# HaploConduct/HaploConduct

Hardware: NVIDIA B200
Metric: candidate_overlaps_scored_per_sec (higher is better)
Workload: dtype u32 fixed-point (2^-22) sums + f64 reference-order pass at threshold boundaries

## Files before the change

### haploconduct_b200/csrc/hc_kernels.cu

```cuda
#include "hc_kernels.cuh"

namespace {

typedef unsigned long long u64;

struct Win {
    u64 xpos;
    uint32_t ypos16;
    uint32_t L;
    uint32_t status;
    uint32_t hasN;
};

struct CandSetup {
    Win w[2];
    uint32_t two;
    uint32_t err;
};

__device__ __forceinline__ hc_candidate load_candidate(const hc_kparams& P, u64 i) {
    hc_candidate c;
    if (P.cand_compact == 4u) {
        const uint16_t* hp = reinterpret_cast<const uint16_t*>(P.cand) + 3 * i;
        const uint32_t h0 = __ldg(hp), h1 = __ldg(hp + 1), h2 = __ldg(hp + 2);
        const uint32_t lo = h0 | (h1 << 16);
        uint32_t r = __ldg(P.tile_run + (i >> 5));
        while ((uint32_t)i >= __ldg(P.run_start + r + 1)) r++;
        const uint32_t anchor = __ldg(P.run_anchor + r), other = lo & 0x01ffffffu;
        const bool anchor_is_2 = ((lo >> 25) & 1u) != 0u;
        c.idx1 = anchor_is_2 ? other : anchor;
        c.idx2 = anchor_is_2 ? anchor : other;
        c.pos1 = (lo >> 30) | ((h2 & 0x7fu) << 2);
        c.pos2 = h2 >> 7;
        c.len1 = c.len2 = 0; c.perc1 = c.perc2 = 0; c.type1 = c.type2 = 0; c.reserved = 0;
        c.ori1 = (lo >> 26) & 1u; c.ori2 = (lo >> 27) & 1u;
        const uint32_t o = (lo >> 28) & 3u;
        c.ord = o == 1 ? '1' : (o == 2 ? '2' : '-');
        return c;
    }
    if (P.cand_compact == 3u) {
        const uint2 e = __ldg(reinterpret_cast<const uint2*>(P.cand) + i);
        uint32_t r = __ldg(P.tile_run + (i >> 5));
        while ((uint32_t)i >= __ldg(P.run_start + r + 1)) r++;
        const uint32_t anchor = __ldg(P.run_anchor + r), other = e.x & 0x7fffffffu;
        const bool anchor_is_2 = (e.x >> 31) != 0u;
        c.idx1 = anchor_is_2 ? other : anchor;
        c.idx2 = anchor_is_2 ? anchor : other;
        const uint32_t w = e.y;
        c.pos1 = w & 0x3fffu; c.pos2 = (w >> 14) & 0x3fffu;
        c.len1 = c.len2 = 0; c.perc1 = c.perc2 = 0; c.type1 = c.type2 = 0; c.reserved = 0;
        c.ori1 = (w >> 28) & 1u; c.ori2 = (w >> 29) & 1u;
        const uint32_t o = w >> 30;
        c.ord = o == 1 ? '1' : (o == 2 ? '2' : '-');
        return c;
    }
    if (P.cand_compact == 2u) {
        const uint32_t* sp = reinterpret_cast<const uint32_t*>(P.cand) + 3 * i;
        const uint32_t w = __ldg(sp + 2);
        c.idx1 = __ldg(sp); c.idx2 = __ldg(sp + 1); c.pos1 = w & 0x3fffu; c.pos2 = (w >> 14) & 0x3fffu;
        c.len1 = c.len2 = 0; c.perc1 = c.perc2 = 0; c.type1 = c.type2 = 0; c.reserved = 0;
        c.ori1 = (w >> 28) & 1u; c.ori2 = (w >> 29) & 1u;
        const uint32_t o = w >> 30;
        c.ord = o == 1 ? '1' : (o == 2 ? '2' : '-');
        return c;
    }
    if (P.cand_compact) {
        const uint4 a = __ldg(reinterpret_cast<const uint4*>(P.cand) + i);
        c.idx1 = a.x; c.idx2 = a.y; c.pos1 = a.z & 0x0fffffffu; c.pos2 = a.w;
        c.len1 = c.len2 = 0; c.perc1 = c.perc2 = 0; c.type1 = c.type2 = 0; c.reserved = 0;
        c.ori1 = (a.z >> 28) & 1u; c.ori2 = (a.z >> 29) & 1u;
        const uint32_t o = a.z >> 30;
        c.ord = o == 1 ? '1' : (o == 2 ? '2' : '-');
        return c;
    }
    const uint4* cp = reinterpret_cast<const uint4*>(P.cand) + 2 * i;
    const uint4 a = __ldg(cp), b = __ldg(cp + 1);
    c.idx1 = a.x; c.idx2 = a.y; c.pos1 = a.z; c.pos2 = a.w;
    c.len1 = b.x; c.len2 = b.y;
    c.perc1 = b.z & 0xff; c.perc2 = (b.z >> 8) & 0xff; c.ord = (b.z >> 16) & 0xff; c.ori1 = (b.z >> 24) & 0xff;
    c.ori2 = b.w & 0xff; c.type1 = (b.w >> 8) & 0xff; c.type2 = (b.w >> 16) & 0xff; c.reserved = 0;
    return c;
}

__device__ __forceinline__ void make_window(const hc_kparams& P, uint32_t rawA, uint32_t slotA, int rcA, uint32_t rawB,
                                            uint32_t slotB, int rcB, uint32_t pos, Win& w) {
    const uint32_t lenA = rawA & HC_LEN_MASK, lenB = rawB & HC_LEN_MASK;
    w.L = 0;
    w.xpos = 0;
    w.ypos16 = 0;
    w.hasN = 0;
    if (pos >= lenA) { w.status = HC_WIN_POS_OOR; return; }
    if (lenA < P.min_read_len || lenB < P.min_read_len) { w.status = HC_WIN_SHORT; return; }
    const u64 sa = 16ull * slotA + (rcA ? hc_slot_size(lenA) : 0u);
    const u64 sb = 16ull * slotB + (rcB ? hc_slot_size(lenB) : 0u);
    w.xpos = sa + pos;
    w.ypos16 = (uint32_t)(sb >> 4);
    w.L = min(lenA - pos, lenB);
    w.status = HC_WIN_SCORED;
    w.hasN = ((rawA | rawB) & HC_HASN_BIT) ? 1u : 0u;
}

__device__ __forceinline__ void setup_windows(const hc_kparams& P, const hc_candidate& c, const uint4& r1, const uint4& r2,
                                              CandSetup& s) {
    const int p1 = (r1.w & HC_LEN_MASK) != 0, p2 = (r2.w & HC_LEN_MASK) != 0;
    const int rc1 = c.ori1 ? 0 : 1, rc2 = c.ori2 ? 0 : 1;
    const int f1 = p1 ? rc1 : 0, s1 = p1 ? 1 - rc1 : 0;
    const int f2 = p2 ? rc2 : 0, s2 = p2 ? 1 - rc2 : 0;
    s.two = (p1 | p2) ? 1u : 0u;
    s.err = 0;
    s.w[1].L = 0; s.w[1].xpos = 0; s.w[1].ypos16 = 0; s.w[1].hasN = 0; s.w[1].status = HC_WIN_UNUSED;
    if (p1 && p2) { if (c.ord != '1' && c.ord != '2') s.err = 1; }
    else if (P.n_single == 0) s.err = 1;
    make_window(P, f1 ? r1.w : r1.z, f1 ? r1.y : r1.x, rc1, f2 ? r2.w : r2.z, f2 ? r2.y : r2.x, rc2, c.pos1, s.w[0]);
    if (s.two) {
        const uint32_t ra = s1 ? r1.w : r1.z, sa = s1 ? r1.y : r1.x;
        const uint32_t rb = s2 ? r2.w : r2.z, sb = s2 ? r2.y : r2.x;
        const bool swapped = p1 && (!p2 || c.ord == '2');
        if (swapped) make_window(P, rb, sb, rc2, ra, sa, rc1, c.pos2, s.w[1]);
        else make_window(P, ra, sa, rc1, rb, sb, rc2, c.pos2, s.w[1]);
    }
    if (s.err) { s.w[0].L = s.w[1].L = 0; s.w[0].status = s.w[1].status = HC_WIN_UNUSED; }
}

__device__ __forceinline__ void extra_pos(const hc_candidate& c, const uint4& r1, const uint4& r2, int32_t& pos3, int32_t& pos4) {
    const uint32_t l10 = r1.z & HC_LEN_MASK, l11 = r1.w & HC_LEN_MASK, l20 = r2.z & HC_LEN_MASK, l21 = r2.w & HC_LEN_MASK;
    const int p1 = l11 != 0, p2 = l21 != 0;
    if (!p1 && !p2) { pos3 = (int32_t)(l10 - c.pos1 - l20); pos4 = 0; }
    else if (!p1) { pos3 = (int32_t)(l10 - c.pos2 - l21); pos4 = (int32_t)(l10 - c.pos1 - l20); }
    else if (!p2) { pos3 = (int32_t)(l11 + c.pos2 - l20); pos4 = (int32_t)(l20 + c.pos1 - l10); }
    else {
        pos3 = c.ord == '1' ? (int32_t)(l11 - c.pos2 - l21) : (int32_t)(l11 + c.pos2 - l21);
        pos4 = (int32_t)(l10 - c.pos1 - l20);
    }
}

__device__ __forceinline__ bool load_and_setup(const hc_kparams& P, const hc_candidate& c, CandSetup& s, uint4& r1, uint4& r2) {
    if (c.idx1 >= P.n_reads || c.idx2 >= P.n_reads || c.idx1 == c.idx2) {
        s.err = 1; s.two = 0;
        s.w[0].L = s.w[1].L = 0; s.w[0].xpos = s.w[1].xpos = 0; s.w[0].ypos16 = s.w[1].ypos16 = 0;
        s.w[0].hasN = s.w[1].hasN = 0; s.w[0].status = s.w[1].status = HC_WIN_UNUSED;
        r1 = r2 = make_uint4(0, 0, 0, 0);
        return false;
    }
    r1 = __ldg(reinterpret_cast<const uint4*>(P.rdesc + c.idx1));
    r2 = __ldg(reinterpret_cast<const uint4*>(P.rdesc + c.idx2));
    setup_windows(P, c, r1, r2, s);
    return !s.err;
}

__device__ __forceinline__ void prefetch_l2(const void* p) { asm volatile("prefetch.global.L2 [%0];" ::"l"(p)); }

__device__ __forceinline__ void prefetch_window(const hc_kparams& P, const Win& w) {
    if (w.L == 0) return;
    const uint32_t n = min(w.L, 512u);
    if (P.packed) {
        const uint8_t* xa = P.pk + (w.xpos & ~127ull);
        const uint32_t xe = (uint32_t)(w.xpos & 127ull) + n;
        for (uint32_t o = 0; o < xe; o += 128) prefetch_l2(xa + o);
        const uint8_t* ya = P.pk + 16ull * w.ypos16;
        for (uint32_t o = 0; o < n; o += 128) prefetch_l2(ya + o);
        return;
    }
    const uint8_t* xa = P.qual + (w.xpos & ~127ull);
    const uint32_t xe = (uint32_t)(w.xpos & 127ull) + n;
    for (uint32_t o = 0; o < xe; o += 128) prefetch_l2(xa + o);
    const uint8_t* ya = P.qual + 16ull * w.ypos16;
    for (uint32_t o = 0; o < n; o += 128) prefetch_l2(ya + o);
    prefetch_l2(P.base2 + (w.xpos >> 4));
    prefetch_l2(P.base2 + ((w.xpos + n) >> 4));
    prefetch_l2(P.base2 + w.ypos16);
}

__device__ __forceinline__ uint32_t prmt(uint32_t a, uint32_t b, uint32_t sel) {
    uint32_t d;
    asm("prmt.b32 %0, %1, %2, %3;" : "=r"(d) : "r"(a), "r"(b), "r"(sel));
    return d;
}

__device__ __forceinline__ void ldg256(const void* p, uint32_t* d) {
    asm("ld.global.nc.v8.u32 {%0,%1,%2,%3,%4,%5,%6,%7}, [%8];"
        : "=r"(d[0]), "=r"(d[1]), "=r"(d[2]), "=r"(d[3]), "=r"(d[4]), "=r"(d[5]), "=r"(d[6]), "=r"(d[7])
        : "l"(p));
}

template <bool HAS_VOID>
__device__ __forceinline__ void lookup16(const uint32_t* __restrict__ T, const uint32_t* wa, const uint32_t* wy, uint32_t m,
                                         uint32_t& acc, uint32_t& orv) {
#pragma unroll
    for (int j = 0; j < 4; j++) {
        const uint32_t mj = (m >> (8 * j)) & 0x55u;
        const uint32_t dep = (mj * 0x02082080u) & 0x80808080u;
        const uint32_t col = (wa[j] ^ hc_swz4(wy[j])) | dep;
        const uint32_t t0 = T[prmt(col, wy[j], 0xCC40u)];
        const uint32_t t1 = T[prmt(col, wy[j], 0xDD51u)];
        const uint32_t t2 = T[prmt(col, wy[j], 0xEE62u)];
        const uint32_t t3 = T[prmt(col, wy[j], 0xFF73u)];
        acc += (t0 + t1) + (t2 + t3);
        if (HAS_VOID) orv |= (t0 | t1) | (t2 | t3);
    }
}

template <bool HAS_VOID>
__device__ __forceinline__ void process32(const hc_kparams& P, const uint32_t* __restrict__ T, u64 xpos, uint32_t ypos16,
                                          uint32_t L, uint32_t hasN, uint32_t k, uint32_t& sum, uint32_t& mm, uint32_t& ncnt,
                                          uint32_t& vd) {
    const u64 xp = xpos + 32ull * k;
    const uint32_t n = min(L - 32u * k, 32u);
    const uint32_t yq = ypos16 + 2u * k;
    const uint32_t off = (uint32_t)xp & 15u;
    const bool two = n > 16u, x1 = off + n > 16u, x2 = off + n > 32u;
    const uint4 z4 = make_uint4(0, 0, 0, 0);
#ifndef HC_NO_LD256
    const uint32_t off32 = (uint32_t)xp & 31u;
    uint32_t QA[16], wy[8];
    const uint8_t* xb = P.qual + (xp & ~31ull);
    ldg256(xb, QA);
    if (off32 + n > 32u) ldg256(xb + 32, QA + 8);
    else {
#pragma unroll
        for (int i = 8; i < 16; i++) QA[i] = 0u;
    }
    ldg256(P.qual + 16ull * yq, wy);
    (void)two; (void)z4;
#else
    const uint4* xq = reinterpret_cast<const uint4*>(P.qual + (xp & ~15ull));
    const uint4 q0 = __ldg(xq);
    const uint4 q1 = x1 ? __ldg(xq + 1) : z4;
    const uint4 q2 = x2 ? __ldg(xq + 2) : z4;
    const uint4* yqp = reinterpret_cast<const uint4*>(P.qual) + yq;
    const uint4 y0 = __ldg(yqp);
    const uint4 y1 = two ? __ldg(yqp + 1) : z4;
#endif
    const uint32_t* bxp = P.base2 + (xp >> 4);
    const uint32_t b0 = __ldg(bxp);
    const uint32_t b1 = x1 ? __ldg(bxp + 1) : 0u;
    const uint32_t b2 = x2 ? __ldg(bxp + 2) : 0u;
    const uint2 by = __ldg(reinterpret_cast<const uint2*>(P.base2 + yq));
    const uint32_t bsh = off * 2u;
    const uint32_t xa0 = __funnelshift_r(b0, b1, bsh) ^ by.x;
    const uint32_t xa1 = __funnelshift_r(b1, b2, bsh) ^ by.y;
    uint32_t m0 = (xa0 | (xa0 >> 1)) & 0x55555555u;
    uint32_t m1 = (xa1 | (xa1 >> 1)) & 0x55555555u;
    if (n < 32u) {
        const uint32_t n0 = min(n, 16u), n1 = n - n0;
        m0 &= n0 >= 16u ? 0xffffffffu : ((1u << (2u * n0)) - 1u);
        m1 &= (1u << (2u * n1)) - 1u;
    }
    ncnt = 0;
    if (hasN) {
        const uint32_t* nap = P.nmask + (xp >> 5);
        const uint32_t na0 = __ldg(nap), na1 = __ldg(nap + 1);
        uint32_t nn = __funnelshift_r(na0, na1, (uint32_t)xp & 31u) | __ldg(P.nmask + (yq >> 1));
        if (n < 32u) nn &= (1u << n) - 1u;
        ncnt = __popc(nn);
        uint32_t s0 = nn & 0xffffu, s1 = nn >> 16;
        s0 = (s0 | (s0 << 8)) & 0x00ff00ffu; s1 = (s1 | (s1 << 8)) & 0x00ff00ffu;
        s0 = (s0 | (s0 << 4)) & 0x0f0f0f0fu; s1 = (s1 | (s1 << 4)) & 0x0f0f0f0fu;
        s0 = (s0 | (s0 << 2)) & 0x33333333u; s1 = (s1 | (s1 << 2)) & 0x33333333u;
        s0 = (s0 | (s0 << 1)) & 0x55555555u; s1 = (s1 | (s1 << 1)) & 0x55555555u;
        m0 &= ~s0;
        m1 &= ~s1;
    }
    mm = __popc(m0) + __popc(m1);
    const bool s2 = (off & 8u) != 0, s1 = (off & 4u) != 0;
    uint32_t V1[10], V[9];
#ifndef HC_NO_LD256
    const bool s4 = (off32 & 16u) != 0;
    uint32_t V2[12];
#pragma unroll
    for (int i = 0; i < 12; i++) V2[i] = s4 ? QA[i + 4] : QA[i];
#pragma unroll
    for (int i = 0; i < 10; i++) V1[i] = s2 ? V2[i + 2] : V2[i];
#else
    const uint32_t W[12] = {q0.x, q0.y, q0.z, q0.w, q1.x, q1.y, q1.z, q1.w, q2.x, q2.y, q2.z, q2.w};
#pragma unroll
    for (int i = 0; i < 10; i++) V1[i] = s2 ? W[i + 2] : W[i];
    const uint32_t wy[8] = {y0.x, y0.y, y0.z, y0.w, y1.x, y1.y, y1.z, y1.w};
#endif
#pragma unroll
    for (int i = 0; i < 9; i++) V[i] = s1 ? V1[i + 1] : V1[i];
    const uint32_t sh = (off & 3u) * 8u;
    uint32_t wa[8];
#pragma unroll
    for (int i = 0; i < 8; i++) wa[i] = __funnelshift_r(V[i], V[i + 1], sh);
    uint32_t acc = 0, orv = 0;
    lookup16<HAS_VOID>(T, wa, wy, m0, acc, orv);
    lookup16<HAS_VOID>(T, wa + 4, wy + 4, m1, acc, orv);
    sum = acc;
    vd = HAS_VOID ? ((orv & HC_VOID_BIT) ? 1u : 0u) : 0u;
}

#ifdef HC_NO_LD256
struct PkRow {
    uint4 q0, q1, q2, y0, y1;
    uint32_t n, off, hasN;
};
#else
struct PkRow {
    uint32_t a[16];
    uint32_t y[8];
    uint32_t n, off, hasN;
};

#endif

__device__ __forceinline__ PkRow load32_packed(const hc_kparams& P, u64 xpos, uint32_t ypos16, uint32_t L, uint32_t hasN, uint32_t k) {
    PkRow r;
    const u64 xp = xpos + 32ull * k;
    r.n = min(L - 32u * k, 32u);
    const uint32_t yq = ypos16 + 2u * k;
    r.hasN = hasN;
#ifndef HC_NO_LD256
    r.off = (uint32_t)xp & 31u;
    const uint8_t* xb = P.pk + (xp & ~31ull);
    ldg256(xb, r.a);
    if (r.off + r.n > 32u) ldg256(xb + 32, r.a + 8);
    else {
#pragma unroll
        for (int i = 8; i < 16; i++) r.a[i] = 0u;
    }
    ldg256(P.pk + 16ull * yq, r.y);
    return r;
#else
    r.off = (uint32_t)xp & 15u;
    const bool two = r.n > 16u, x1 = r.off + r.n > 16u, x2 = r.off + r.n > 32u;
    const uint4 z4 = make_uint4(0, 0, 0, 0);
    const uint4* xq = reinterpret_cast<const uint4*>(P.pk + (xp & ~15ull));
    r.q0 = __ldg(xq);
    r.q1 = x1 ? __ldg(xq + 1) : z4;
    r.q2 = x2 ? __ldg(xq + 2) : z4;
    const uint4* yqp = reinterpret_cast<const uint4*>(P.pk) + yq;
    r.y0 = __ldg(yqp);
    r.y1 = two ? __ldg(yqp + 1) : z4;
    return r;
#endif
}

template <bool HAS_VOID>
__device__ __forceinline__ void compute32_packed(const uint32_t* __restrict__ T, const uint32_t* __restrict__ VM, const PkRow& r,
                                                 uint32_t& sum, uint32_t& mm, uint32_t& ncnt, uint32_t& vd) {
    const uint32_t n = r.n, off = r.off, hasN = r.hasN;
    const uint32_t vm = VM[n];
#ifndef HC_NO_LD256
    const bool s4 = (off & 16u) != 0, s2 = (off & 8u) != 0, s1 = (off & 4u) != 0;
    uint32_t V2[12], V1[10], V[9];
#pragma unroll
    for (int i = 0; i < 12; i++) V2[i] = s4 ? r.a[i + 4] : r.a[i];
#pragma unroll
    for (int i = 0; i < 10; i++) V1[i] = s2 ? V2[i + 2] : V2[i];
#pragma unroll
    for (int i = 0; i < 9; i++) V[i] = s1 ? V1[i + 1] : V1[i];
    const uint32_t sh = (off & 3u) * 8u;
    const uint32_t* wy = r.y;
#else
    const uint4 q0 = r.q0, q1 = r.q1, q2 = r.q2, y0 = r.y0, y1 = r.y1;
    const uint32_t W[12] = {q0.x, q0.y, q0.z, q0.w, q1.x, q1.y, q1.z, q1.w, q2.x, q2.y, q2.z, q2.w};
    const bool s2 = (off & 8u) != 0, s1 = (off & 4u) != 0;
    uint32_t V1[10], V[9];
#pragma unroll
    for (int i = 0; i < 10; i++) V1[i] = s2 ? W[i + 2] : W[i];
#pragma unroll
    for (int i = 0; i < 9; i++) V[i] = s1 ? V1[i + 1] : V1[i];
    const uint32_t sh = (off & 3u) * 8u;
    const uint32_t wy[8] = {y0.x, y0.y, y0.z, y0.w, y1.x, y1.y, y1.z, y1.w};
#endif
    uint32_t acc = 0, orv = 0, flags = 0, vw = 0;
#pragma unroll
    for (int j = 0; j < 8; j++) {
        const uint32_t wa = __funnelshift_r(V[j], V[j + 1], sh);
        const uint32_t wb = wy[j];
        const uint32_t col = wa ^ hc_swz4_packed(wb);
        const uint32_t row = wb & 0x3f3f3f3fu;
        flags |= ((col | (col << 1)) & 0x80808080u) >> j;
        if (hasN) {
            const uint32_t nzA = (((wa & 0x7f7f7f7fu) + 0x7f7f7f7fu) | wa), nzB = (((wb & 0x7f7f7f7fu) + 0x7f7f7f7fu) | wb);
            vw |= ((nzA & nzB) & 0x80808080u) >> j;
        }
        const uint32_t t0 = T[prmt(col, row, 0xCC40u)];
        const uint32_t t1 = T[prmt(col, row, 0xDD51u)];
        const uint32_t t2 = T[prmt(col, row, 0xEE62u)];
        const uint32_t t3 = T[prmt(col, row, 0xFF73u)];
        acc += (t0 + t1) + (t2 + t3);
        if (HAS_VOID) orv |= (t0 | t1) | (t2 | t3);
    }
    ncnt = 0;
    if (hasN) {
        const uint32_t valid = vw & vm;
        ncnt = n - __popc(valid);
        flags &= valid;
    } else {
        flags &= vm;
    }
    mm = __popc(flags);
    sum = acc;
    vd = HAS_VOID ? ((orv & HC_VOID_BIT) ? 1u : 0u) : 0u;
}

template <bool HAS_VOID>
__device__ __forceinline__ void process32_packed(const hc_kparams& P, const uint32_t* __restrict__ T,
                                                 const uint32_t* __restrict__ VM, u64 xpos, uint32_t ypos16, uint32_t L,
                                                 uint32_t hasN, uint32_t k, uint32_t& sum, uint32_t& mm, uint32_t& ncnt,
                                                 uint32_t& vd) {
    const PkRow r = load32_packed(P, xpos, ypos16, L, hasN, k);
    compute32_packed<HAS_VOID>(T, VM, r, sum, mm, ncnt, vd);
}

template <bool HAS_VOID, bool PACKED>
__device__ __forceinline__ void process_chunk(const hc_kparams& P, const uint32_t* __restrict__ T, const uint32_t* __restrict__ VM,
                                              u64 xpos, uint32_t ypos16, uint32_t L, uint32_t hasN, uint32_t k, uint32_t& sum,
                                              uint32_t& mm, uint32_t& ncnt, uint32_t& vd) {
    if (PACKED) process32_packed<HAS_VOID>(P, T, VM, xpos, ypos16, L, hasN, k, sum, mm, ncnt, vd);
    else process32<HAS_VOID>(P, T, xpos, ypos16, L, hasN, k, sum, mm, ncnt, vd);
}

__device__ __forceinline__ uint32_t warp_incl_scan(uint32_t v, int lane) {
#pragma unroll
    for (int d = 1; d < 32; d <<= 1) {
        uint32_t t = __shfl_up_sync(0xffffffffu, v, d);
        if (lane >= d) v += t;
    }
    return v;
}

struct WinAcc {
    u64 S;
    uint32_t mm;
    uint32_t nn;
    uint32_t vd;
};

__device__ __forceinline__ double window_mm_rate(uint32_t mm, uint32_t tl) {
    if (tl == 0u) return 1.0;
    return mm ? (double)(float)(int)mm / (double)tl : 0.0;
}

__device__ __forceinline__ uint32_t classify(const hc_kparams& P, uint32_t two, const uint32_t mmc[2], const uint32_t cmp[2],
                                             const int ae[2], const int ao[2]) {
    int both, ov_ok;
    if (two) {
        both = ae[0] && ae[1];
        ov_ok = ao[0] && ao[1];
    } else {
        both = ae[0];
        ov_ok = ao[0];
    }
    uint32_t cls;
    if (both) cls = HC_CLASS_EDGE;
    else {
        bool low;
        if (P.merge_contigs_sign == 0) low = cmp[0] != 0u && mmc[0] == 0u && (!two || (cmp[1] != 0u && mmc[1] == 0u));
        else if (P.merge_contigs_sign < 0) low = false;
        else {
            const double r0 = window_mm_rate(mmc[0], cmp[0]), r1 = window_mm_rate(mmc[1], cmp[1]);
            low = (two ? fmax(r0, r1) : r0) <= P.merge_contigs;
        }
        if (low) cls = HC_CLASS_EDGE;
        else if (ov_ok) cls = HC_CLASS_NONEDGE;
        else cls = HC_CLASS_DISCARD;
    }
    return cls | (both ? HC_CLS_BOTH : 0u);
}

__device__ __forceinline__ double combine_score(uint32_t two, uint32_t both, double ov0, double ov1) {
    if (!two) return ov0;
    return both ? 0.5 * (ov0 + ov1) : fmin(ov0, ov1);
}

__device__ __forceinline__ double fx_mean(u64 S, uint32_t tl) { return -((double)S * (1.0 / HC_FX_SCALE)) / (double)tl; }

__device__ __noinline__ void write_per_cand(const hc_kparams& P, u64 i, double score, double mmrate, uint32_t cls,
                                            const uint32_t mmc[2], const uint32_t cmp[2], const uint32_t st[2], uint32_t exact) {
    hc_result r;
    r.score = score;
    r.mismatch_rate = mmrate;
    const hc_candidate c = load_candidate(P, i);
    uint4 r1 = make_uint4(0, 0, 0, 0), r2 = r1;
    if (c.idx1 < P.n_reads && c.idx2 < P.n_reads) {
        r1 = __ldg(reinterpret_cast<const uint4*>(P.rdesc + c.idx1));
        r2 = __ldg(reinterpret_cast<const uint4*>(P.rdesc + c.idx2));
    }
    extra_pos(c, r1, r2, r.pos3, r.pos4);
    r.mismatches[0] = mmc[0];
    r.mismatches[1] = mmc[1];
    r.compared[0] = cmp[0];
    r.compared[1] = cmp[1];
    r.cls = (uint8_t)(cls & HC_CLS_MASK);
    r.status[0] = (uint8_t)st[0];
    r.status[1] = (uint8_t)st[1];
    r.exact = (uint8_t)exact;
    r.indel_count = 0;
    P.per_cand[i] = r;
}

template <bool HAS_VOID, bool PACKED>
__global__ void __launch_bounds__(HC_WARPS_MAX * 32, HC_MIN_CTAS) hc_score_kernel(const hc_kparams P) {
    extern __shared__ __align__(16) unsigned char smem[];
    uint32_t* T = reinterpret_cast<uint32_t*>(smem);
    const uint32_t ntab = (P.ncodes + 1u) * 256u;
    uint32_t* VM = T + ntab;
    for (uint32_t i = threadIdx.x; i < ntab; i += blockDim.x) T[i] = P.fx_table[i];
    if (threadIdx.x < HC_VM_WORDS) VM[threadIdx.x] = hc_packed_vmask(threadIdx.x);
    __syncthreads();

    const int lane = threadIdx.x & 31;
    const int warp = threadIdx.x >> 5;
    const int nwarps = blockDim.x >> 5;
    unsigned char* scratch = smem + (size_t)(ntab + HC_VM_WORDS) * 4u + (size_t)warp * HC_WARP_SCRATCH;
    uint2* part = reinterpret_cast<uint2*>(scratch);
    uint4* wdA = reinterpret_cast<uint4*>(scratch + HC_PARTMAX * 8u);
    uint2* wdB = reinterpret_cast<uint2*>(scratch + HC_PARTMAX * 8u + HC_WINSLOTS * 16u);
    uint32_t* head = reinterpret_cast<uint32_t*>(scratch + HC_PARTMAX * 8u + HC_WINSLOTS * 24u);

    const u64 ntiles = (P.n + 31ull) >> 5;
    const u64 gwarp = (u64)blockIdx.x * nwarps + warp;
    const u64 twarps = (u64)gridDim.x * nwarps;
    const uint32_t lane_le = 0xffffffffu >> (31 - lane);

    uint32_t st_windows = 0, st_positions = 0, st_bytes = 0, st_errors = 0;

    for (u64 tile = gwarp; tile < ntiles; tile += twarps) {
        const u64 i = (tile << 5) + lane;
        const bool valid = i < P.n;
        CandSetup s;
        s.err = 0; s.two = 0;
        s.w[0].L = s.w[1].L = 0; s.w[0].status = s.w[1].status = HC_WIN_UNUSED;
        s.w[0].xpos = s.w[1].xpos = 0; s.w[0].ypos16 = s.w[1].ypos16 = 0; s.w[0].hasN = s.w[1].hasN = 0;
        if (valid) {
            const hc_candidate c = load_candidate(P, i);
            uint4 r1, r2;
            load_and_setup(P, c, s, r1, r2);
#ifndef HC_NO_PREFETCH
            prefetch_window(P, s.w[0]);
            prefetch_window(P, s.w[1]);
#endif
        }
        WinAcc acc[2];
        acc[0].S = acc[1].S = 0; acc[0].mm = acc[1].mm = 0; acc[0].nn = acc[1].nn = 0; acc[0].vd = acc[1].vd = 0;
        const uint32_t c0 = (s.w[0].L + 31u) >> 5, c1 = (s.w[1].L + 31u) >> 5;
        const uint32_t ct = c0 + c1;

        uint32_t bigmask = __ballot_sync(0xffffffffu, ct >= HC_BIG_CHUNKS);
        while (bigmask) {
            const int src = __ffs(bigmask) - 1;
            bigmask &= bigmask - 1;
#pragma unroll
            for (int w = 0; w < 2; w++) {
                const uint32_t xl = __shfl_sync(0xffffffffu, (uint32_t)s.w[w].xpos, src);
                const uint32_t xh = __shfl_sync(0xffffffffu, (uint32_t)(s.w[w].xpos >> 32), src);
                const uint32_t yp = __shfl_sync(0xffffffffu, s.w[w].ypos16, src);
                const uint32_t Lw = __shfl_sync(0xffffffffu, s.w[w].L, src);
                const uint32_t hn = __shfl_sync(0xffffffffu, s.w[w].hasN, src);
                const uint32_t cw = (Lw + 31u) >> 5;
                if (cw == 0) continue;
                const u64 xpos = ((u64)xh << 32) | xl;
                u64 S = 0;
                uint32_t mm = 0, nn = 0, vd = 0;
                for (uint32_t k = lane; k < cw; k += 32) {
                    uint32_t sum, m1, n1, v1;
                    process_chunk<HAS_VOID, PACKED>(P, T, VM, xpos, yp, Lw, hn, k, sum, m1, n1, v1);
                    S += sum; mm += m1; nn += n1; vd |= v1;
                }
#pragma unroll
                for (int d = 16; d > 0; d >>= 1) {
                    S += __shfl_xor_sync(0xffffffffu, S, d);
                    mm += __shfl_xor_sync(0xffffffffu, mm, d);
                    nn += __shfl_xor_sync(0xffffffffu, nn, d);
                    vd |= __shfl_xor_sync(0xffffffffu, vd, d);
                }
                if (lane == src) { acc[w].S = S; acc[w].mm = mm; acc[w].nn = nn; acc[w].vd = vd; }
            }
        }

        uint32_t pending = __ballot_sync(0xffffffffu, ct > 0 && ct < HC_BIG_CHUNKS);
        while (pending) {
            const bool mine = (pending >> lane) & 1u;
            const uint32_t nwin = (c0 > 0) + (c1 > 0);
            const uint32_t v = mine ? (ct | (nwin << 16)) : 0u;
            const uint32_t incl = warp_incl_scan(v, lane);
            const bool fit = mine && ((incl & 0xffffu) <= HC_PARTMAX);
            const uint32_t take = __ballot_sync(0xffffffffu, fit);
            const int last = 31 - __clz(take);
            const uint32_t C = __shfl_sync(0xffffffffu, incl, last) & 0xffffu;
            if (lane < (int)(HC_PARTMAX / 32u)) head[lane] = 0;
            __syncwarp();
            uint32_t start0 = 0, start1 = 0;
            if (fit) {
                start0 = (incl & 0xffffu) - ct;
                start1 = start0 + c0;
                uint32_t slot = (incl >> 16) - nwin;
                if (c0) {
                    wdA[slot] = make_uint4((uint32_t)s.w[0].xpos, (uint32_t)(s.w[0].xpos >> 32), s.w[0].ypos16, s.w[0].L);
                    wdB[slot] = make_uint2(start0, s.w[0].hasN);
                    atomicOr(&head[start0 >> 5], 1u << (start0 & 31u));
                    slot++;
                }
                if (c1) {
                    wdA[slot] = make_uint4((uint32_t)s.w[1].xpos, (uint32_t)(s.w[1].xpos >> 32), s.w[1].ypos16, s.w[1].L);
                    wdB[slot] = make_uint2(start1, s.w[1].hasN);
                    atomicOr(&head[start1 >> 5], 1u << (start1 & 31u));
                }
            }
            __syncwarp();
            uint32_t running = 0;
            for (uint32_t f0 = 0; f0 < C; f0 += 32) {
                const uint32_t hw = head[f0 >> 5];
                const uint32_t f = f0 + lane;
                if (f < C) {
                    const uint32_t slot = running + __popc(hw & lane_le) - 1u;
                    const uint4 a = wdA[slot];
                    const uint2 b = wdB[slot];
                    uint32_t sum, m1, n1, v1;
                    process_chunk<HAS_VOID, PACKED>(P, T, VM, ((u64)a.y << 32) | a.x, a.z, a.w, b.y, f - b.x, sum, m1, n1, v1);
                    part[f] = make_uint2(sum, m1 | (n1 << 12) | (v1 << 24));
                }
                running += __popc(hw);
            }
            __syncwarp();
            if (fit) {
                u64 S = 0;
                uint32_t pk = 0;
                for (uint32_t k = 0; k < c0; k++) { const uint2 e = part[start0 + k]; S += e.x; pk += e.y; }
                if (c0) { acc[0].S = S; acc[0].mm = pk & 0xfffu; acc[0].nn = (pk >> 12) & 0xfffu; acc[0].vd = pk >> 24; }
                S = 0; pk = 0;
                for (uint32_t k = 0; k < c1; k++) { const uint2 e = part[start1 + k]; S += e.x; pk += e.y; }
                if (c1) { acc[1].S = S; acc[1].mm = pk & 0xfffu; acc[1].nn = (pk >> 12) & 0xfffu; acc[1].vd = pk >> 24; }
            }
            __syncwarp();
            pending &= ~take;
        }

        bool flag = false;
        if (valid) {
            if (s.err) {
                st_errors++;
                P.cls[i] = HC_CLASS_DISCARD;
                if (P.per_cand) {
                    const uint32_t z[2] = {0, 0};
                    const uint32_t stt[2] = {HC_WIN_UNUSED, HC_WIN_UNUSED};
                    write_per_cand(P, i, 0.0, 1.0, HC_CLASS_DISCARD, z, z, stt, 0);
                }
            } else {
                int ae[2], ao[2];
                uint32_t mmc[2] = {0, 0}, cmp[2] = {0, 0}, stt[2];
#pragma unroll
                for (int w = 0; w < 2; w++) {
                    uint32_t status = s.w[w].status;
                    ae[w] = P.zero_above_edge;
                    ao[w] = P.zero_above_ov;
                    if (status == HC_WIN_SCORED) {
                        const uint32_t tl = s.w[w].L - acc[w].nn;
                        if (acc[w].vd) {
                            status = HC_WIN_VOID;
                            if (P.void_exact) flag = true;
                        } else if (tl == 0) {
                            status = HC_WIN_EMPTY;
                        } else {
                            cmp[w] = tl;
                            mmc[w] = acc[w].mm;
                            const double dl = (double)tl, dS = (double)acc[w].S;
                            const bool up_e = !P.never_edge && (dS <= P.ce_up * dl);
                            const bool dn_e = P.never_edge || (dS > P.ce_dn * dl);
                            const bool up_o = !P.never_ov && (dS <= P.co_up * dl);
                            const bool dn_o = P.never_ov || (dS > P.co_dn * dl);
                            ae[w] = up_e;
                            ao[w] = up_o;
                            if (!(up_e || dn_e) || !(up_o || dn_o)) flag = true;
                        }
                        st_windows++;
                        st_positions += s.w[w].L;
                        st_bytes += 2u * ((s.w[w].L + 3u) >> 2) + 2u * ((s.w[w].L + 7u) >> 3) + 2u * s.w[w].L;
                    }
                    stt[w] = status;
                }
                st_bytes += 48;
                const uint32_t cls = classify(P, s.two, mmc, cmp, ae, ao);
                if (P.exact_edges && (cls & HC_CLS_MASK) == HC_CLASS_EDGE) flag = true;
                P.cls[i] = (uint8_t)cls;
                if ((cls & HC_CLS_MASK) == HC_CLASS_EDGE) {
                    hc_tmp32 t;
                    t.S[0] = acc[0].S; t.S[1] = acc[1].S;
                    t.tl[0] = cmp[0]; t.tl[1] = cmp[1];
                    t.mm[0] = mmc[0]; t.mm[1] = mmc[1];
                    P.tmp[i] = t;
                }
                if (P.per_cand) {
                    const double ov0 = cmp[0] ? exp(fx_mean(acc[0].S, cmp[0])) : 0.0;
                    const double ov1 = cmp[1] ? exp(fx_mean(acc[1].S, cmp[1])) : 0.0;
                    const double r0 = window_mm_rate(mmc[0], cmp[0]), r1 = window_mm_rate(mmc[1], cmp[1]);
                    write_per_cand(P, i, combine_score(s.two, cls & HC_CLS_BOTH, ov0, ov1), s.two ? fmax(r0, r1) : r0, cls, mmc, cmp, stt, 0);
                }
            }
        }
        const uint32_t fm = __ballot_sync(0xffffffffu, flag);
        if (fm) {
            unsigned long long base = 0;
            if (lane == 0) base = atomicAdd(&P.counters[HC_CNT_FLAGGED], (unsigned long long)__popc(fm));
            base = __shfl_sync(0xffffffffu, base, 0);
            if (flag) P.flagged[base + __popc(fm & (lane_le >> 1))] = (uint32_t)i;
        }
    }
#pragma unroll
    for (int d = 16; d > 0; d >>= 1) {
        st_errors += __shfl_xor_sync(0xffffffffu, st_errors, d);
    }
    u64 w_windows = st_windows, w_positions = st_positions, w_bytes = st_bytes;
#pragma unroll
    for (int d = 16; d > 0; d >>= 1) {
        w_windows += __shfl_xor_sync(0xffffffffu, w_windows, d);
        w_positions += __shfl_xor_sync(0xffffffffu, w_positions, d);
        w_bytes += __shfl_xor_sync(0xffffffffu, w_bytes, d);
    }
    if (lane == 0) {
        atomicAdd(&P.counters[HC_CNT_WINDOWS], w_windows);
        atomicAdd(&P.counters[HC_CNT_POSITIONS], w_positions);
        atomicAdd(&P.counters[HC_CNT_ALGBYTES], w_bytes);
        if (st_errors) atomicAdd(&P.counters[HC_CNT_ERRORS], (unsigned long long)st_errors);
    }
}

__device__ void exact_window(const hc_kparams& P, const double* __restrict__ sdbl, const Win& w, double& mean, double& mmrate, uint32_t& mmc,
                             uint32_t& cmp, uint32_t& status) {
    mean = 0.0;
    mmrate = 1.0;
    mmc = 0;
    cmp = 0;
    status = w.status;
    if (w.status != HC_WIN_SCORED) return;
    const uint32_t n1 = P.ncodes + 1u;
    double total = 0.0;
    uint32_t tl = 0, mm = 0;
    const u64 yp = 16ull * w.ypos16;
    if (P.packed) {
        const uint32_t nblk = (w.L + 31u) >> 5;
        for (uint32_t k = 0; k < nblk; k++) {
            const PkRow r = load32_packed(P, w.xpos, w.ypos16, w.L, 0u, k);
            const bool s4 = (r.off & 16u) != 0, s2 = (r.off & 8u) != 0, s1 = (r.off & 4u) != 0;
            uint32_t V2[12], V1[10], V[9];
#pragma unroll
            for (int i = 0; i < 12; i++) V2[i] = s4 ? r.a[i + 4] : r.a[i];
#pragma unroll
            for (int i = 0; i < 10; i++) V1[i] = s2 ? V2[i + 2] : V2[i];
#pragma unroll
            for (int i = 0; i < 9; i++) V[i] = s1 ? V1[i + 1] : V1[i];
            const uint32_t sh = (r.off & 3u) * 8u;
#pragma unroll
            for (uint32_t j = 0; j < 32; j++) {
                if (j < r.n) {
                    const uint32_t wa = __funnelshift_r(V[j >> 2], V[(j >> 2) + 1], sh);
                    const uint32_t a = (wa >> (8 * (j & 3))) & 0xffu, b = (r.y[j >> 2] >> (8 * (j & 3))) & 0xffu;
                    if (a != 0 && b != 0) {
                        const uint32_t mis = (a >> 6) != (b >> 6);
                        mm += mis;
                        const uint32_t ti = hc_dbl_index(a & 63u, b & 63u, mis, n1);
                        const double lp = sdbl ? sdbl[ti] : __ldg(P.dbl_table + ti);
                        if (lp > 0.0) { status = HC_WIN_VOID; return; }
                        total = __dadd_rn(total, lp);
                        tl++;
                    }
                }
            }
        }
    } else {
        for (uint32_t i = 0; i < w.L; i++) {
            const u64 xa = w.xpos + i, xb = yp + i;
            const uint32_t nA = (P.nmask[xa >> 5] >> (xa & 31)) & 1u, nB = (P.nmask[xb >> 5] >> (xb & 31)) & 1u;
            if (nA | nB) continue;
            const uint32_t a = (P.base2[xa >> 4] >> (2 * (xa & 15))) & 3u, b = (P.base2[xb >> 4] >> (2 * (xb & 15))) & 3u;
            const uint32_t mis = a != b;
            mm += mis;
            const double lp = P.dbl_table[hc_dbl_index(P.qual[xa], P.qual[xb], mis, n1)];
            if (lp > 0.0) { status = HC_WIN_VOID; return; }
            total = __dadd_rn(total, lp);
            tl++;
        }
    }
    if (tl == 0) { status = HC_WIN_EMPTY; return; }
    mmc = mm;
    cmp = tl;
    const double dl = (double)tl;
    mmrate = __ddiv_rn((double)(float)(int)mm, dl);
    mean = __dmul_rn(__ddiv_rn(1.0, dl), total);
}

__device__ void exact_window_wide(const hc_kparams& P, const double* __restrict__ T2, const Win& w, double& mean, double& mmrate,
                                  uint32_t& mmc, uint32_t& cmp, uint32_t& status) {
    mean = 0.0;
    mmrate = 1.0;
    mmc = 0;
    cmp = 0;
    status = w.status;
    if (w.status != HC_WIN_SCORED) return;
    double total = 0.0;
    uint32_t tl = 0, mm = 0;
    const uint32_t nblk = (w.L + 31u) >> 5;
    for (uint32_t k = 0; k < nblk; k++) {
        const PkRow r = load32_packed(P, w.xpos, w.ypos16, w.L, 0u, k);
        const bool s4 = (r.off & 16u) != 0, s2 = (r.off & 8u) != 0, s1 = (r.off & 4u) != 0;
        uint32_t V2[12], V1[10], V[9];
#pragma unroll
        for (int i = 0; i < 12; i++) V2[i] = s4 ? r.a[i + 4] : r.a[i];
#pragma unroll
        for (int i = 0; i < 10; i++) V1[i] = s2 ? V2[i + 2] : V2[i];
#pragma unroll
        for (int i = 0; i < 9; i++) V[i] = s1 ? V1[i + 1] : V1[i];
        const uint32_t sh = (r.off & 3u) * 8u;
        uint32_t flags = 0, vw = 0;
        bool vd = false;
#pragma unroll
        for (int j = 0; j < 8; j++) {
            const uint32_t wa = __funnelshift_r(V[j], V[j + 1], sh), wb = r.y[j];
            const uint32_t x = wa ^ wb;
            const uint32_t mf = (x | (x << 1)) & 0x80808080u;
            const uint32_t col = (wa & 0x3f3f3f3fu) | mf, row = wb & 0x3f3f3f3fu;
            const uint32_t nzA = (((wa & 0x7f7f7f7fu) + 0x7f7f7f7fu) | wa), nzB = (((wb & 0x7f7f7f7fu) + 0x7f7f7f7fu) | wb);
            flags |= mf >> j;
            vw |= ((nzA & nzB) & 0x80808080u) >> j;
            const double l0 = T2[prmt(col, row, 0xCC40u)], l1 = T2[prmt(col, row, 0xDD51u)];
            const double l2 = T2[prmt(col, row, 0xEE62u)], l3 = T2[prmt(col, row, 0xFF73u)];
            vd = vd || l0 > 0.0 || l1 > 0.0 || l2 > 0.0 || l3 > 0.0;
            total = __dadd_rn(total, l0);
            total = __dadd_rn(total, l1);
            total = __dadd_rn(total, l2);
            total = __dadd_rn(total, l3);
        }
        if (vd) { status = HC_WIN_VOID; return; }
        tl += __popc(vw);
        mm += __popc(flags & vw);
    }
    if (tl == 0) { status = HC_WIN_EMPTY; return; }
    mmc = mm;
    cmp = tl;
    const double dl = (double)tl;
    mmrate = __ddiv_rn((double)(float)(int)mm, dl);
    mean = __dmul_rn(__ddiv_rn(1.0, dl), total);
}

__device__ void exact_window_warp(const hc_kparams& P, const Win& w, int lane, double& mean, double& mmrate, uint32_t& mmc,
                                  uint32_t& cmp, uint32_t& status) {
    mean = 0.0;
    mmrate = 1.0;
    mmc = 0;
    cmp = 0;
    status = w.status;
    if (w.status != HC_WIN_SCORED) return;
    const uint32_t n1 = P.ncodes + 1u;
    double total = 0.0;
    uint32_t tl = 0, mm = 0;
    const u64 yp = 16ull * w.ypos16;
    for (uint32_t i0 = 0; i0 < w.L; i0 += 32) {
        const uint32_t i = i0 + lane;
        bool valid = false;
        uint32_t mis = 0;
        double lp = 0.0;
        if (i < w.L) {
            const u64 xa = w.xpos + i, xb = yp + i;
            if (P.packed) {
                const uint32_t a = P.pk[xa], b = P.pk[xb];
                if (a != 0 && b != 0) {
                    valid = true;
                    mis = (a >> 6) != (b >> 6);
                    lp = __ldg(P.dbl_table + hc_dbl_index(a & 63u, b & 63u, mis, n1));
                }
            } else {
                const uint32_t nA = (P.nmask[xa >> 5] >> (xa & 31)) & 1u, nB = (P.nmask[xb >> 5] >> (xb & 31)) & 1u;
                if (!(nA | nB)) {
                    valid = true;
                    const uint32_t a = (P.base2[xa >> 4] >> (2 * (xa & 15))) & 3u, b = (P.base2[xb >> 4] >> (2 * (xb & 15))) & 3u;
                    mis = a != b;
                    lp = P.dbl_table[hc_dbl_index(P.qual[xa], P.qual[xb], mis, n1)];
                }
            }
        }
        const uint32_t vmask = __ballot_sync(0xffffffffu, valid);
        const uint32_t mmask = __ballot_sync(0xffffffffu, valid && mis);
        if (__any_sync(0xffffffffu, valid && lp > 0.0)) { status = HC_WIN_VOID; return; }
        mm += __popc(mmask);
        tl += __popc(vmask);
        for (uint32_t rem = vmask; rem; rem &= rem - 1)
            total = __dadd_rn(total, __shfl_sync(0xffffffffu, lp, __ffs(rem) - 1));
    }
    if (tl == 0) { status = HC_WIN_EMPTY; return; }
    mmc = mm;
    cmp = tl;
    const double dl = (double)tl;
    mmrate = __ddiv_rn((double)(float)(int)mm, dl);
    mean = __dmul_rn(__ddiv_rn(1.0, dl), total);
}

__global__ void hc_exact_kernel(const hc_kparams P, uint32_t table_in_smem) {
    extern __shared__ __align__(16) unsigned char smem[];
    const u64 nf = P.counters[HC_CNT_FLAGGED];
    const u64 nthreads = (u64)gridDim.x * blockDim.x;
    const bool warp_mode = nf * 32ull <= nthreads;
    const double* sdbl = nullptr;
    const double* swide = nullptr;
    if (table_in_smem == 1u && !warp_mode && nf > 0) {
        double* t = reinterpret_cast<double*>(smem);
        const uint32_t nent = (P.ncodes + 1u) * (P.ncodes + 1u) * 2u;
        for (uint32_t k = threadIdx.x; k < nent; k += blockDim.x) t[k] = P.dbl_table[k];
        __syncthreads();
        sdbl = t;
    }
    if (table_in_smem == 2u && !warp_mode && nf > 0) {
        double* t = reinterpret_cast<double*>(smem);
        const uint32_t n1 = P.ncodes + 1u, nent = n1 * 256u;
        for (uint32_t k = threadIdx.x; k < nent; k += blockDim.x) {
            const uint32_t b = k >> 8, a = k & 63u, m = (k >> 7) & 1u;
            t[k] = (a == 0u || b == 0u || a >= n1 || (k & 64u)) ? 0.0 : P.dbl_table[hc_dbl_index(a, b, m, n1)];
        }
        __syncthreads();
        swide = t;
    }
    const int lane = threadIdx.x & 31;
    const u64 tid = (u64)blockIdx.x * blockDim.x + threadIdx.x;
    const bool writer = !warp_mode || lane == 0;
    for (u64 t = warp_mode ? tid >> 5 : tid; t < nf; t += warp_mode ? nthreads >> 5 : nthreads) {
        const u64 i = P.flagged[t];
        const hc_candidate c = load_candidate(P, i);
        CandSetup s;
        uint4 r1, r2;
        if (!load_and_setup(P, c, s, r1, r2)) continue;
        double mean[2], mmr[2] = {1.0, 1.0};
        int ae[2], ao[2];
        uint32_t mmc[2], cmp[2], stt[2];
#pragma unroll
        for (int w = 0; w < 2; w++) {
            if (warp_mode) exact_window_warp(P, s.w[w], lane, mean[w], mmr[w], mmc[w], cmp[w], stt[w]);
            else if (swide) exact_window_wide(P, swide, s.w[w], mean[w], mmr[w], mmc[w], cmp[w], stt[w]);
// ... 380 lines not shown
```

Measured before the change: 4.869 billion.

## Align packed chunk scoring to anchor-read 32-byte rows and batch lanes by row

Windows now record an anchor offset, so in the packed path each 32-position chunk is aligned to the anchor read's 32-byte grid. The partner read is loaded at an arbitrary offset and shifted into place with funnel shifts. When few distinct anchor rows are present, lanes working on the same row index are grouped together so their anchor loads hit the same cache lines. The intended gain is aligned, shared loads for the anchor read instead of two unaligned loads per chunk. The cost is possibly one extra chunk per window, more complex shuffling and reduction logic, and reuse of the head array as a row-slot buffer.

```diff
diff --git a/haploconduct_b200/csrc/hc_kernels.cu b/haploconduct_b200/csrc/hc_kernels.cu
--- a/haploconduct_b200/csrc/hc_kernels.cu
+++ b/haploconduct_b200/csrc/hc_kernels.cu
@@ -10,7 +10,10 @@
     uint32_t L;
     uint32_t status;
     uint32_t hasN;
+    uint32_t aoff;
 };
+
+#define HC_AOFF_B 0x80000000u
 
 struct CandSetup {
     Win w[2];
@@ -83,12 +86,13 @@
 }
 
 __device__ __forceinline__ void make_window(const hc_kparams& P, uint32_t rawA, uint32_t slotA, int rcA, uint32_t rawB,
-                                            uint32_t slotB, int rcB, uint32_t pos, Win& w) {
+                                            uint32_t slotB, int rcB, uint32_t pos, bool anchorA, Win& w) {
     const uint32_t lenA = rawA & HC_LEN_MASK, lenB = rawB & HC_LEN_MASK;
     w.L = 0;
     w.xpos = 0;
     w.ypos16 = 0;
     w.hasN = 0;
+    w.aoff = anchorA ? pos : HC_AOFF_B;
     if (pos >= lenA) { w.status = HC_WIN_POS_OOR; return; }
     if (lenA < P.min_read_len || lenB < P.min_read_len) { w.status = HC_WIN_SHORT; return; }
     const u64 sa = 16ull * slotA + (rcA ? hc_slot_size(lenA) : 0u);
@@ -108,16 +112,17 @@
     const int f2 = p2 ? rc2 : 0, s2 = p2 ? 1 - rc2 : 0;
     s.two = (p1 | p2) ? 1u : 0u;
     s.err = 0;
-    s.w[1].L = 0; s.w[1].xpos = 0; s.w[1].ypos16 = 0; s.w[1].hasN = 0; s.w[1].status = HC_WIN_UNUSED;
+    s.w[1].L = 0; s.w[1].xpos = 0; s.w[1].ypos16 = 0; s.w[1].hasN = 0; s.w[1].aoff = 0; s.w[1].status = HC_WIN_UNUSED;
     if (p1 && p2) { if (c.ord != '1' && c.ord != '2') s.err = 1; }
     else if (P.n_single == 0) s.err = 1;
-    make_window(P, f1 ? r1.w : r1.z, f1 ? r1.y : r1.x, rc1, f2 ? r2.w : r2.z, f2 ? r2.y : r2.x, rc2, c.pos1, s.w[0]);
+    const bool first1 = c.idx1 < c.idx2;
+    make_window(P, f1 ? r1.w : r1.z, f1 ? r1.y : r1.x, rc1, f2 ? r2.w : r2.z, f2 ? r2.y : r2.x, rc2, c.pos1, first1, s.w[0]);
     if (s.two) {
         const uint32_t ra = s1 ? r1.w : r1.z, sa = s1 ? r1.y : r1.x;
         const uint32_t rb = s2 ? r2.w : r2.z, sb = s2 ? r2.y : r2.x;
         const bool swapped = p1 && (!p2 || c.ord == '2');
-        if (swapped) make_window(P, rb, sb, rc2, ra, sa, rc1, c.pos2, s.w[1]);
-        else make_window(P, ra, sa, rc1, rb, sb, rc2, c.pos2, s.w[1]);
+        if (swapped) make_window(P, rb, sb, rc2, ra, sa, rc1, c.pos2, !first1, s.w[1]);
+        else make_window(P, ra, sa, rc1, rb, sb, rc2, c.pos2, first1, s.w[1]);
     }
     if (s.err) { s.w[0].L = s.w[1].L = 0; s.w[0].status = s.w[1].status = HC_WIN_UNUSED; }
 }
@@ -138,7 +143,7 @@
     if (c.idx1 >= P.n_reads || c.idx2 >= P.n_reads || c.idx1 == c.idx2) {
         s.err = 1; s.two = 0;
         s.w[0].L = s.w[1].L = 0; s.w[0].xpos = s.w[1].xpos = 0; s.w[0].ypos16 = s.w[1].ypos16 = 0;
-        s.w[0].hasN = s.w[1].hasN = 0; s.w[0].status = s.w[1].status = HC_WIN_UNUSED;
+        s.w[0].hasN = s.w[1].hasN = 0; s.w[0].aoff = s.w[1].aoff = 0; s.w[0].status = s.w[1].status = HC_WIN_UNUSED;
         r1 = r2 = make_uint4(0, 0, 0, 0);
         return false;
     }
@@ -405,6 +410,75 @@
     compute32_packed<HAS_VOID>(T, VM, r, sum, mm, ncnt, vd);
 }
 
+template <bool HAS_VOID>
+__device__ __forceinline__ void chunk_anchor_packed(const hc_kparams& P, const uint32_t* __restrict__ T, const uint32_t* __restrict__ VM,
+                                                    u64 ppos, uint32_t aslot16, uint32_t o, uint32_t L, uint32_t hasN, uint32_t k,
+                                                    uint32_t& sum, uint32_t& mm, uint32_t& ncnt, uint32_t& vd) {
+    const uint32_t lo = 32u * k < o ? o - 32u * k : 0u;
+    const uint32_t hi = min(o + L - 32u * k, 32u);
+    uint32_t y[8], a[16];
+    ldg256(P.pk + 16ull * aslot16 + 32ull * k, y);
+    const long long xp = (long long)ppos + 32ll * k - (long long)o;
+    const uint32_t off = (uint32_t)xp & 31u;
+    const uint8_t* xb = P.pk + (xp & ~31ll);
+    ldg256(xb, a);
+    if (off + hi > 32u) ldg256(xb + 32, a + 8);
+    else {
+#pragma unroll
+        for (int i = 8; i < 16; i++) a[i] = 0u;
+    }
+    const bool s4 = (off & 16u) != 0, s2 = (off & 8u) != 0, s1 = (off & 4u) != 0;
+    uint32_t V2[12], V1[10], V[9];
+#pragma unroll
+    for (int i = 0; i < 12; i++) V2[i] = s4 ? a[i + 4] : a[i];
+#pragma unroll
+    for (int i = 0; i < 10; i++) V1[i] = s2 ? V2[i + 2] : V2[i];
+#pragma unroll
+    for (int i = 0; i < 9; i++) V[i] = s1 ? V1[i + 1] : V1[i];
+    const uint32_t sh = (off & 3u) * 8u;
+    const uint32_t rv = VM[hi] & ~VM[lo];
+    uint32_t acc = 0, orv = 0, flags = 0, vw = 0;
+#pragma unroll
+    for (int j = 0; j < 8; j++) {
+        const uint32_t bm = prmt(rv << j, 0u, 0xBA98u);
+        const uint32_t wp = __funnelshift_r(V[j], V[j + 1], sh) & bm;
+        const uint32_t wn = y[j] & bm;
+        const uint32_t col = wp ^ hc_swz4_packed(wn);
+        const uint32_t row = wn & 0x3f3f3f3fu;
+        flags |= ((col | (col << 1)) & 0x80808080u) >> j;
+        if (hasN) {
+            const uint32_t nzP = (((wp & 0x7f7f7f7fu) + 0x7f7f7f7fu) | wp), nzN = (((wn & 0x7f7f7f7fu) + 0x7f7f7f7fu) | wn);
+            vw |= ((nzP & nzN) & 0x80808080u) >> j;
+        }
+        const uint32_t t0 = T[prmt(col, row, 0xCC40u)];
+        const uint32_t t1 = T[prmt(col, row, 0xDD51u)];
+        const uint32_t t2 = T[prmt(col, row, 0xEE62u)];
+        const uint32_t t3 = T[prmt(col, row, 0xFF73u)];
+        acc += (t0 + t1) + (t2 + t3);
+        if (HAS_VOID) orv |= (t0 | t1) | (t2 | t3);
+    }
+    ncnt = 0;
+    if (hasN) {
+        ncnt = (hi - lo) - __popc(vw);
+        flags &= vw;
+    }
+    mm = __popc(flags);
+    sum = acc;
+    vd = HAS_VOID ? ((orv & HC_VOID_BIT) ? 1u : 0u) : 0u;
+}
+
+__device__ __forceinline__ uint32_t anchor_off(const Win& w) { return (w.aoff & HC_AOFF_B) ? 0u : w.aoff; }
+__device__ __forceinline__ uint32_t anchor_chunks(const Win& w) {
+    const uint32_t o = anchor_off(w);
+    return w.L ? ((o + w.L - 1u) >> 5) - (o >> 5) + 1u : 0u;
+}
+
+__device__ __forceinline__ void anchor_rows(const Win& w, bool fit, uint32_t cw, uint32_t& kmin, uint32_t& kend) {
+    const uint32_t kf = anchor_off(w) >> 5;
+    kmin = __reduce_min_sync(0xffffffffu, fit && cw ? kf : 0xffffffffu);
+    kend = __reduce_max_sync(0xffffffffu, fit && cw ? kf + cw : 0u);
+}
+
 template <bool HAS_VOID, bool PACKED>
 __device__ __forceinline__ void process_chunk(const hc_kparams& P, const uint32_t* __restrict__ T, const uint32_t* __restrict__ VM,
                                               u64 xpos, uint32_t ypos16, uint32_t L, uint32_t hasN, uint32_t k, uint32_t& sum,
@@ -525,6 +599,7 @@
         s.err = 0; s.two = 0;
         s.w[0].L = s.w[1].L = 0; s.w[0].status = s.w[1].status = HC_WIN_UNUSED;
         s.w[0].xpos = s.w[1].xpos = 0; s.w[0].ypos16 = s.w[1].ypos16 = 0; s.w[0].hasN = s.w[1].hasN = 0;
+        s.w[0].aoff = s.w[1].aoff = 0;
         if (valid) {
             const hc_candidate c = load_candidate(P, i);
             uint4 r1, r2;
@@ -572,58 +647,109 @@
         }
 
         uint32_t pending = __ballot_sync(0xffffffffu, ct > 0 && ct < HC_BIG_CHUNKS);
+        const uint32_t cw0 = PACKED ? anchor_chunks(s.w[0]) : c0, cw1 = PACKED ? anchor_chunks(s.w[1]) : c1;
+        const uint32_t cwt = cw0 + cw1;
         while (pending) {
             const bool mine = (pending >> lane) & 1u;
-            const uint32_t nwin = (c0 > 0) + (c1 > 0);
-            const uint32_t v = mine ? (ct | (nwin << 16)) : 0u;
+            const uint32_t nwin = (cw0 > 0) + (cw1 > 0);
+            const uint32_t v = mine ? (cwt | (nwin << 16)) : 0u;
             const uint32_t incl = warp_incl_scan(v, lane);
             const bool fit = mine && ((incl & 0xffffu) <= HC_PARTMAX);
             const uint32_t take = __ballot_sync(0xffffffffu, fit);
             const int last = 31 - __clz(take);
             const uint32_t C = __shfl_sync(0xffffffffu, incl, last) & 0xffffu;
+            uint32_t rows = 0;
+            if (PACKED) {
+#pragma unroll
+                for (int w = 0; w < 2; w++) {
+                    uint32_t kmin, kend;
+                    anchor_rows(s.w[w], fit, w ? cw1 : cw0, kmin, kend);
+                    rows += kend > kmin ? kend - kmin : 0u;
+                }
+            }
+            const bool by_anchor = PACKED && 2u * rows <= 3u * ((C + 31u) >> 5);
             if (lane < (int)(HC_PARTMAX / 32u)) head[lane] = 0;
             __syncwarp();
-            uint32_t start0 = 0, start1 = 0;
+            uint32_t start0 = 0, start1 = 0, slot0 = 0;
             if (fit) {
-                start0 = (incl & 0xffffu) - ct;
-                start1 = start0 + c0;
-                uint32_t slot = (incl >> 16) - nwin;
-                if (c0) {
-                    wdA[slot] = make_uint4((uint32_t)s.w[0].xpos, (uint32_t)(s.w[0].xpos >> 32), s.w[0].ypos16, s.w[0].L);
-                    wdB[slot] = make_uint2(start0, s.w[0].hasN);
-                    atomicOr(&head[start0 >> 5], 1u << (start0 & 31u));
+                start0 = (incl & 0xffffu) - cwt;
+                start1 = start0 + cw0;
+                slot0 = (incl >> 16) - nwin;
+                uint32_t slot = slot0;
+#pragma unroll
+                for (int w = 0; w < 2; w++) {
+                    const uint32_t cw = w ? cw1 : cw0, start = w ? start1 : start0;
+                    if (!cw) continue;
+                    const Win& W = s.w[w];
+                    if (PACKED) {
+                        const bool ab = (W.aoff & HC_AOFF_B) != 0;
+                        const uint32_t o = anchor_off(W);
+                        const u64 pp = ab ? W.xpos : 16ull * W.ypos16;
+                        const uint32_t as16 = ab ? W.ypos16 : (uint32_t)((W.xpos - o) >> 4);
+                        wdA[slot] = make_uint4((uint32_t)pp, (uint32_t)(pp >> 32), as16, W.L);
+                        wdB[slot] = make_uint2(start, W.hasN | (o << 1));
+                    } else {
+                        wdA[slot] = make_uint4((uint32_t)W.xpos, (uint32_t)(W.xpos >> 32), W.ypos16, W.L);
+                        wdB[slot] = make_uint2(start, W.hasN);
+                    }
+                    if (!by_anchor) atomicOr(&head[start >> 5], 1u << (start & 31u));
                     slot++;
-                }
-                if (c1) {
-                    wdA[slot] = make_uint4((uint32_t)s.w[1].xpos, (uint32_t)(s.w[1].xpos >> 32), s.w[1].ypos16, s.w[1].L);
-                    wdB[slot] = make_uint2(start1, s.w[1].hasN);
-                    atomicOr(&head[start1 >> 5], 1u << (start1 & 31u));
                 }
             }
             __syncwarp();
-            uint32_t running = 0;
-            for (uint32_t f0 = 0; f0 < C; f0 += 32) {
-                const uint32_t hw = head[f0 >> 5];
-                const uint32_t f = f0 + lane;
-                if (f < C) {
-                    const uint32_t slot = running + __popc(hw & lane_le) - 1u;
-                    const uint4 a = wdA[slot];
-                    const uint2 b = wdB[slot];
-                    uint32_t sum, m1, n1, v1;
-                    process_chunk<HAS_VOID, PACKED>(P, T, VM, ((u64)a.y << 32) | a.x, a.z, a.w, b.y, f - b.x, sum, m1, n1, v1);
-                    part[f] = make_uint2(sum, m1 | (n1 << 12) | (v1 << 24));
+            if (by_anchor) {
+                uint8_t* row_slot = reinterpret_cast<uint8_t*>(head);
+#pragma unroll
+                for (int w = 0; w < 2; w++) {
+                    const uint32_t kf = anchor_off(s.w[w]) >> 5, cw = fit ? (w ? cw1 : cw0) : 0u;
+                    const uint32_t my_slot = slot0 + (w ? (cw0 > 0) : 0u);
+                    for (uint32_t k = __reduce_min_sync(0xffffffffu, cw ? kf : 0xffffffffu); __any_sync(0xffffffffu, cw && k < kf + cw); k++) {
+                        const bool covers = k - kf < cw;
+                        const uint32_t mask = __ballot_sync(0xffffffffu, covers);
+                        if (!mask) continue;
+                        if (covers) row_slot[__popc(mask & (lane_le >> 1))] = (uint8_t)my_slot;
+                        __syncwarp();
+                        if (lane < __popc(mask)) {
+                            const uint32_t slot = row_slot[lane];
+                            const uint4 a = wdA[slot];
+                            const uint2 b = wdB[slot];
+                            uint32_t sum, m1, n1, v1;
+                            chunk_anchor_packed<HAS_VOID>(P, T, VM, ((u64)a.y << 32) | a.x, a.z, b.y >> 1, a.w, b.y & 1u, k,
+                                                          sum, m1, n1, v1);
+                            part[b.x + k - (b.y >> 6)] = make_uint2(sum, m1 | (n1 << 12) | (v1 << 24));
+                        }
+                        __syncwarp();
+                    }
                 }
-                running += __popc(hw);
+            } else {
+                uint32_t running = 0;
+                for (uint32_t f0 = 0; f0 < C; f0 += 32) {
+                    const uint32_t hw = head[f0 >> 5];
+                    const uint32_t f = f0 + lane;
+                    if (f < C) {
+                        const uint32_t slot = running + __popc(hw & lane_le) - 1u;
+                        const uint4 a = wdA[slot];
+                        const uint2 b = wdB[slot];
+                        uint32_t sum, m1, n1, v1;
+                        if (PACKED) chunk_anchor_packed<HAS_VOID>(P, T, VM, ((u64)a.y << 32) | a.x, a.z, b.y >> 1, a.w, b.y & 1u,
+                                                                  (b.y >> 6) + (f - b.x), sum, m1, n1, v1);
+                        else process_chunk<HAS_VOID, PACKED>(P, T, VM, ((u64)a.y << 32) | a.x, a.z, a.w, b.y, f - b.x, sum, m1, n1, v1);
+                        part[f] = make_uint2(sum, m1 | (n1 << 12) | (v1 << 24));
+                    }
+                    running += __popc(hw);
+                }
             }
             __syncwarp();
             if (fit) {
+                start0 = wdB[slot0].x;
+                start1 = start0 + cw0;
                 u64 S = 0;
                 uint32_t pk = 0;
-                for (uint32_t k = 0; k < c0; k++) { const uint2 e = part[start0 + k]; S += e.x; pk += e.y; }
-                if (c0) { acc[0].S = S; acc[0].mm = pk & 0xfffu; acc[0].nn = (pk >> 12) & 0xfffu; acc[0].vd = pk >> 24; }
+                for (uint32_t k = 0; k < cw0; k++) { const uint2 e = part[start0 + k]; S += e.x; pk += e.y; }
+                if (cw0) { acc[0].S = S; acc[0].mm = pk & 0xfffu; acc[0].nn = (pk >> 12) & 0xfffu; acc[0].vd = pk >> 24; }
                 S = 0; pk = 0;
-                for (uint32_t k = 0; k < c1; k++) { const uint2 e = part[start1 + k]; S += e.x; pk += e.y; }
-                if (c1) { acc[1].S = S; acc[1].mm = pk & 0xfffu; acc[1].nn = (pk >> 12) & 0xfffu; acc[1].vd = pk >> 24; }
+                for (uint32_t k = 0; k < cw1; k++) { const uint2 e = part[start1 + k]; S += e.x; pk += e.y; }
+                if (cw1) { acc[1].S = S; acc[1].mm = pk & 0xfffu; acc[1].nn = (pk >> 12) & 0xfffu; acc[1].vd = pk >> 24; }
             }
             __syncwarp();
             pending &= ~take;
```

Result: slower. 2.134 billion, median of 6 (-56.2%).
